# SamsungLabs/nb-asr

Measured on AMD Instinct MI355X. Metric: utterances_per_sec, higher is better.
Workload: dtype f32

## Files before the change

### include/nbasr.h

```cpp
#ifndef NBASR_H
#define NBASR_H

#include <stddef.h>

#ifdef __cplusplus
extern "C" {
#endif

#define NBASR_ABI_VERSION 6

#define NBASR_OK 0
#define NBASR_EINVAL (-1)
#define NBASR_EALIGN (-2)
#define NBASR_ENULL (-3)

typedef void* nbasr_stream_t;

#define NBASR_F32 0
#define NBASR_BF16 1

int nbasr_version(void);

const char* nbasr_build_id(void);

// ... 11 lines not shown
    const float* beta;
} nbasr_deferred_ln;

int nbasr_layernorm_channels(const void* x, const float* gamma, const float* beta, void* y, float* absmax,
                             int batch, int channels, int frames, int ld, float eps, int in_dtype, int out_dtype,
                             nbasr_stream_t stream);

int nbasr_dense_conv1d_fused(const float* x, const float* w, const float* bias,
                             const float* skip0, const float* skip1, const float* skip2,
                             float* y, int batch, int c_in, int frames_in, int ld_in,
                             int c_out, int ld_out, int kernel, int stride,
                             const nbasr_deferred_ln* ln, int ln_on_x, int ln_on_skip0, nbasr_stream_t stream);

#define NBASR_DENSE_STATS_UNIT 16
#define NBASR_DENSE_BF16X3 0
#define NBASR_DENSE_F16X2 1
#define NBASR_DENSE_BF16 2
size_t nbasr_packed_dense_weights_bytes(int scheme, int c_out, int c_in, int kernel, int row_tile);
int nbasr_pack_dense_weights(int scheme, const float* w, void* packed, int c_out, int c_in, int kernel, int stride, int row_tile,
                             nbasr_stream_t stream);
int nbasr_dense_conv1d_packed(int scheme, const void* x, int x_is_image, const float* x_absmax, const float* x_range,
                              const void* packed_w, const float* bias,
                              const float* skip0, const float* skip1, const float* skip2, void* y,
                              int batch, int c_in, int frames_in, int ld_in, int c_out, int ld_out, int kernel, int stride,
                              int row_tile, int frame_tile, const nbasr_deferred_ln* ln, float* stats_part, nbasr_stream_t stream);
int nbasr_input_range(const float* x, float* range, int batch, int channels, int frames, int ld, nbasr_stream_t stream);

size_t nbasr_split_image_bytes(int batch, int channels, int ld);
int nbasr_layernorm_split_image(const float* x, const float* gamma, const float* beta, float* stats, float* bound,
                                void* image, int batch, int channels, int frames, int ld, float eps,
                                nbasr_stream_t stream);
int nbasr_split_image_ranged(const float* x, const float* x_range, void* image, int batch, int channels, int frames, int ld,
                             nbasr_stream_t stream);

int nbasr_lstm_input_projection(const float* x, const float* w_ih, const float* b_ih, const float* b_hh,
                                float* gates_ws, int batch, int c_in, int frames, int ld, int hidden,
                                const nbasr_deferred_ln* ln, nbasr_stream_t stream);
size_t nbasr_lstm_packed_whh_bytes(int hidden);
int nbasr_lstm_pack_whh(const float* w_hh, void* packed, int hidden, nbasr_stream_t stream);
int nbasr_lstm_recurrence_packed(const float* gates_ws, const void* packed_whh, float* cell_ws, float* h_out,
                                 int batch, int frames, int hidden, nbasr_stream_t stream);
#define NBASR_LSTM_SEQ_INJECT_FAULT 1
size_t nbasr_lstm_seq_workspace_bytes(int batch, int hidden);
int nbasr_lstm_recurrence_seq(const float* gates_ws, const void* packed_whh, float* cell_ws, float* h_out, void* seq_ws,
                              int batch, int frames, int hidden, int flags, nbasr_stream_t stream);
int nbasr_lstm_seq_status(const void* seq_ws, nbasr_stream_t stream);
size_t nbasr_lstm_packed_whh16_bytes(int hidden);
int nbasr_lstm_pack_whh16(const float* w_hh, void* packed, int hidden, nbasr_stream_t stream);
size_t nbasr_lstm_xcd_workspace_bytes(int batch, int hidden);
int nbasr_lstm_recurrence_xcd(const float* gates_ws, const void* packed_whh16, float* cell_ws, float* h_out, void* xcd_ws,
                              int batch, int frames, int hidden, int flags, nbasr_stream_t stream);
int nbasr_lstm_recurrence_frames16(const float* gates_ws, const void* packed_whh16, float* cell_ws, float* h_out, void* xcd_ws,
                                   int batch, int frames, int hidden, nbasr_stream_t stream);
#define NBASR_LSTM_CONTINUE 2
int nbasr_lstm_recurrence_frames16_state(const float* gates_ws, const void* packed_whh16, float* cell_ws, float* h_out, void* xcd_ws,
                                         const float* h0, int batch, int frames, int hidden, int flags, nbasr_stream_t stream);

int nbasr_linear_head(const float* h, const float* w, const float* bias, float* logits,
                      int rows, int features, int classes, nbasr_stream_t stream);

int nbasr_linear_head_bct(const float* x, const float* w, const float* bias, float* logits,
                          int batch, int features, int frames, int ld, int classes,
                          const nbasr_deferred_ln* ln, nbasr_stream_t stream);

int nbasr_channel_stats(const void* x, float* stats, int batch, int channels, int frames, int ld, float eps, int dtype,
                        nbasr_stream_t stream);
// ... 141 lines not shown
```

### nb_asr_amd/csrc/layernorm.hip

```cpp
#include "storage.h"

namespace nbasr {

constexpr int LN_ROWS = 16;
constexpr int LN_QS = 16;

template <typename T, bool MINMAX = false, int FR = Chunk<T>::FR>
__device__ __forceinline__ void tile_statistics(const T* x, int channels, int ld, float eps, size_t base, bool active,
                                                int row, int ql, float (*s_mean)[LN_QS * FR], float (*s_m2)[LN_QS * FR],
                                                float* s_cnt, float* s_mu, float* s_rstd,
                                                float (*s_lo)[LN_QS * FR] = nullptr, float (*s_hi)[LN_QS * FR] = nullptr)
{
    float shift[FR], s1[FR], s2[FR], lo[FR], hi[FR];
#pragma unroll
    for (int r = 0; r < FR; ++r) { shift[r] = 0.f; s1[r] = 0.f; s2[r] = 0.f; lo[r] = 3.0e38f; hi[r] = -3.0e38f; }
    int n = 0;
    if (active && row < channels) {
        load_frames<FR>(x + base + static_cast<size_t>(row) * ld, shift);
        auto fold = [&](const float (&e)[FR]) {
#pragma unroll
            for (int r = 0; r < FR; ++r) {
                const float d = e[r] - shift[r];
                s1[r] += d;
                s2[r] = __builtin_fmaf(d, d, s2[r]);
// ... 158 lines not shown
    NBASR_REQUIRE(x && gamma && beta && y, NBASR_ENULL, "%s: NULL pointer", what);
    NBASR_REQUIRE(aligned16(x) && aligned16(y), NBASR_EALIGN, "%s: x, y must be 16-byte aligned", what);
    NBASR_REQUIRE(batch <= 65535, NBASR_EINVAL, "%s: batch %d > 65535", what, batch);
    NBASR_REQUIRE(!absmax || in_dtype == NBASR_F32, NBASR_EINVAL, "%s: the absmax by-product exists for fp32 tensors only", what);
    const int nq = ld / fr;
    const dim3 grid((nq + LN_QS - 1) / LN_QS, batch);
    if (in_dtype == NBASR_BF16) {
        if (out_dtype == NBASR_BF16)
            hipLaunchKernelGGL((layernorm_channels_kernel<bf16_t, bf16_t, false>), grid, dim3(256), 0, as_stream(stream),
                               static_cast<const bf16_t*>(x), gamma, beta, static_cast<bf16_t*>(y), channels, frames, ld, eps, static_cast<unsigned*>(nullptr));
        else
            hipLaunchKernelGGL((layernorm_channels_kernel<bf16_t, float, false>), grid, dim3(256), 0, as_stream(stream),
                               static_cast<const bf16_t*>(x), gamma, beta, static_cast<float*>(y), channels, frames, ld, eps, static_cast<unsigned*>(nullptr));
    } else if (absmax) {
        zero_async(absmax, sizeof(float) * batch, as_stream(stream));
        hipLaunchKernelGGL((layernorm_channels_kernel<float, float, true>), grid, dim3(256), 0, as_stream(stream),
                           static_cast<const float*>(x), gamma, beta, static_cast<float*>(y), channels, frames, ld, eps, reinterpret_cast<unsigned*>(absmax));
    } else {
        hipLaunchKernelGGL((layernorm_channels_kernel<float, float, false>), grid, dim3(256), 0, as_stream(stream),
                           static_cast<const float*>(x), gamma, beta, static_cast<float*>(y), channels, frames, ld, eps, static_cast<unsigned*>(nullptr));
    }
    return launch_status(what);
}

extern "C" int nbasr_layernorm_channels(const void* x, const float* gamma, const float* beta, void* y, float* absmax, int batch,
                                        int channels, int frames, int ld, float eps, int in_dtype, int out_dtype, nbasr_stream_t stream)
{
    clear_error();
    NBASR_REQUIRE(!absmax || (in_dtype == NBASR_F32 && out_dtype == NBASR_F32), NBASR_EINVAL,
                  "nbasr_layernorm_channels: the max|y| by-product exists for fp32 -> fp32 only");
    return layernorm_impl("nbasr_layernorm_channels", x, gamma, beta, y, absmax, batch, channels, frames, ld, eps, stream, in_dtype, out_dtype);
}

__global__ __launch_bounds__(256) void channel_stats_bound_kernel(const float* __restrict__ x, const float* __restrict__ gamma,
                                                                  const float* __restrict__ beta, float* __restrict__ stats,
                                                                  unsigned* __restrict__ bound, int channels, int frames, int ld, float eps)
{
    __shared__ float s_mean[LN_ROWS][LN_QS * 4];
    __shared__ float s_m2[LN_ROWS][LN_QS * 4];
    __shared__ float s_cnt[LN_ROWS];
    __shared__ float s_mu[LN_QS * 4];
    __shared__ float s_rstd[LN_QS * 4];
    __shared__ float s_gb[8];
    __shared__ float s_lo[LN_ROWS][LN_QS * 4];
    __shared__ float s_hi[LN_ROWS][LN_QS * 4];

    const int ql = threadIdx.x & (LN_QS - 1);
    const int row = threadIdx.x / LN_QS;
    const int nq = ld >> 2;
    const int q = blockIdx.x * LN_QS + ql;
    const int b = blockIdx.y;
    const bool active = q < nq;
    const size_t base = static_cast<size_t>(b) * channels * ld + static_cast<size_t>(q) * 4;

    float gm = 0.f, bm = 0.f;
    for (int c = threadIdx.x; c < channels; c += 256) { gm = fmaxf(gm, fabsf(gamma[c])); bm = fmaxf(bm, fabsf(beta[c])); }
#pragma unroll
    for (int d = 32; d >= 1; d >>= 1) { gm = fmaxf(gm, __shfl_xor(gm, d)); bm = fmaxf(bm, __shfl_xor(bm, d)); }
    if ((threadIdx.x & 63) == 0) { s_gb[threadIdx.x >> 6] = gm; s_gb[4 + (threadIdx.x >> 6)] = bm; }

    tile_statistics<float, true>(x, channels, ld, eps, base, active, row, ql, s_mean, s_m2, s_cnt, s_mu, s_rstd, s_lo, s_hi);
    gm = fmaxf(fmaxf(s_gb[0], s_gb[1]), fmaxf(s_gb[2], s_gb[3]));
    bm = fmaxf(fmaxf(s_gb[4], s_gb[5]), fmaxf(s_gb[6], s_gb[7]));

    float dev = 0.f;
    if (threadIdx.x < LN_QS * 4) {
        const int t = blockIdx.x * (LN_QS * 4) + threadIdx.x;
        if (t < ld) {
            const bool live = t < frames;
            float* srow = stats + static_cast<size_t>(b) * 2 * ld;
            srow[t] = live ? s_mu[threadIdx.x] : 0.f;
            srow[ld + t] = live ? s_rstd[threadIdx.x] : 0.f;
            if (live) dev = finite_abs(fmaxf(s_hi[0][threadIdx.x] - s_mu[threadIdx.x], s_mu[threadIdx.x] - s_lo[0][threadIdx.x]) * s_rstd[threadIdx.x]);
        }
    }
    if (threadIdx.x < 64) {
#pragma unroll
        for (int d = 32; d >= 1; d >>= 1) dev = fmaxf(dev, __shfl_xor(dev, d));
        if (threadIdx.x == 0) atomicMax(bound + b, __float_as_uint(finite_abs((dev * gm + bm) * 1.0001f)));
    }
}

template <bool NORM>
__global__ __launch_bounds__(256) void normalize_split_kernel(const float* __restrict__ x, const float* __restrict__ stats,
                                                              const float* __restrict__ gamma, const float* __restrict__ beta,
                                                              const float* __restrict__ bound, unsigned char* __restrict__ image,
                                                              int channels, int , int ld,
                                                              int bound_stride)
{
    typedef _Float16 halfx8 __attribute__((ext_vector_type(8)));
    const int ql = threadIdx.x & 63, oct0 = (threadIdx.x >> 6) + 4 * blockIdx.z;
    const int nq = ld >> 2;
    const int q = blockIdx.x * 64 + ql;
    const int b = blockIdx.y;
    const int n_groups = (channels + 15) >> 4;
    const size_t rows = static_cast<size_t>(ld) + 1;
    unsigned char* const img_b = image + static_cast<size_t>(b) * n_groups * 4 * rows * 16;
    if (blockIdx.x == 0 && blockIdx.z == 0) {
        const uint4 z = make_uint4(0u, 0u, 0u, 0u);
        for (int pl = threadIdx.x; pl < n_groups * 4; pl += 256) *reinterpret_cast<uint4*>(img_b + static_cast<size_t>(pl) * rows * 16) = z;
    }
    if (q >= nq) return;
    float scale = 1.f;
    {
        const unsigned bits = __float_as_uint(bound[static_cast<size_t>(b) * bound_stride]);
        const int e = static_cast<int>((bits >> 23) & 0xffu);
        int k = (bits & 0x7fffffffu) ? (127 + 14) - e : 0;
        k = k > 126 ? 126 : (k < -126 ? -126 : k);
        scale = __uint_as_float(static_cast<unsigned>(127 + k) << 23);
    }
    float m4[4] = {0.f, 0.f, 0.f, 0.f}, r4[4] = {0.f, 0.f, 0.f, 0.f};
    if constexpr (NORM) {
        const float* st = stats + static_cast<size_t>(b) * 2 * ld + q * 4;
        const float4 mu = *reinterpret_cast<const float4*>(st), rs = *reinterpret_cast<const float4*>(st + ld);
        m4[0] = mu.x; m4[1] = mu.y; m4[2] = mu.z; m4[3] = mu.w;
        r4[0] = rs.x; r4[1] = rs.y; r4[2] = rs.z; r4[3] = rs.w;
    }
    const float* xb = x + static_cast<size_t>(b) * channels * ld + static_cast<size_t>(q) * 4;
    const int n_oct = (channels + 7) >> 3;
    for (int oct = oct0; oct < 2 * n_groups; oct += 4 * gridDim.z) {
        float v[8][4];
#pragma unroll
        for (int c = 0; c < 8; ++c) {
            const int ch = oct * 8 + c;
            float4 t4 = make_float4(0.f, 0.f, 0.f, 0.f);
            float g = 0.f, be = 0.f;
            if (oct < n_oct && ch < channels) {
                t4 = *reinterpret_cast<const float4*>(xb + static_cast<size_t>(ch) * ld);
                if constexpr (NORM) { g = gamma[ch]; be = beta[ch]; }
            }
            const float e4[4] = {t4.x, t4.y, t4.z, t4.w};
#pragma unroll
            for (int r = 0; r < 4; ++r) {
                if constexpr (NORM) v[c][r] = (ch < channels) ? ln_apply(e4[r], m4[r], r4[r], g, be) * scale : 0.f;
                else                v[c][r] = e4[r] * scale;
            }
        }
        unsigned char* plane_hi = img_b + ((static_cast<size_t>(oct >> 1) * 4 + (oct & 1)) * rows + 1 + static_cast<size_t>(q) * 4) * 16;
        unsigned char* plane_lo = plane_hi + 2 * rows * 16;
#pragma unroll
        for (int r = 0; r < 4; ++r) {
            halfx8 hi, lo;
#pragma unroll
            for (int c = 0; c < 8; ++c) {
                const _Float16 h = static_cast<_Float16>(v[c][r]);
                hi[c] = h;
                lo[c] = static_cast<_Float16>(v[c][r] - static_cast<float>(h));
            }
            *reinterpret_cast<halfx8*>(plane_hi + r * 16) = hi;
            *reinterpret_cast<halfx8*>(plane_lo + r * 16) = lo;
        }
    }
}

static int split_grid_z(int tiles, int batch)
{
    const long long wgs = static_cast<long long>(tiles) * batch;
    int z = 4;
    while (z < 16 && wgs * z < 512) z *= 2;
    return z;
}

extern "C" int nbasr_layernorm_split_image(const float* x, const float* gamma, const float* beta, float* stats, float* bound,
                                           void* image, int batch, int channels, int frames, int ld, float eps,
                                           nbasr_stream_t stream)
{
    clear_error();
    NBASR_REQUIRE(batch >= 0 && channels > 0 && frames >= 0, NBASR_EINVAL, "nbasr_layernorm_split_image: bad sizes");
    NBASR_REQUIRE(ld >= frames && ld % 4 == 0, NBASR_EALIGN, "nbasr_layernorm_split_image: ld=%d must be >= frames=%d and a multiple of 4", ld, frames);
    if (batch == 0 || ld == 0) return NBASR_OK;
    NBASR_REQUIRE(x && gamma && beta && stats && bound && image, NBASR_ENULL, "nbasr_layernorm_split_image: NULL pointer");
    NBASR_REQUIRE(aligned16(x) && aligned16(stats) && aligned16(image), NBASR_EALIGN, "nbasr_layernorm_split_image: x, stats, image must be 16-byte aligned");
    NBASR_REQUIRE(batch <= 65535, NBASR_EINVAL, "nbasr_layernorm_split_image: batch %d > 65535", batch);
    zero_async(bound, sizeof(float) * batch, as_stream(stream));
    const int nq = ld / 4;
    hipLaunchKernelGGL(channel_stats_bound_kernel, dim3((nq + LN_QS - 1) / LN_QS, batch), dim3(256), 0, as_stream(stream),
                       x, gamma, beta, stats, reinterpret_cast<unsigned*>(bound), channels, frames, ld, eps);
    hipLaunchKernelGGL(normalize_split_kernel<true>, dim3((nq + 63) / 64, batch, split_grid_z((nq + 63) / 64, batch)), dim3(256), 0, as_stream(stream),
                       x, stats, gamma, beta, bound, static_cast<unsigned char*>(image), channels, frames, ld, 1);
    return launch_status("nbasr_layernorm_split_image");
}

__global__ __launch_bounds__(256) void input_range_kernel(const float* __restrict__ x, unsigned* __restrict__ range,
                                                          int channels, int frames, int ld)
{
    __shared__ float s_max[4][256];
    __shared__ unsigned s_bad[4];
    const int b = blockIdx.y;
    const int lane = threadIdx.x & 63, slice = threadIdx.x >> 6;
    const int t0 = (blockIdx.x * 64 + lane) * 4;
    float m[4] = {0.f, 0.f, 0.f, 0.f};
    unsigned bad = 0u;
    if (t0 < frames) {
        const float* col = x + static_cast<size_t>(b) * channels * ld + t0;
        const bool whole = t0 + 4 <= ld && ld % 4 == 0 && (reinterpret_cast<size_t>(x) & 15) == 0;
        for (int c = slice; c < channels; c += 4) {
            float v[4] = {0.f, 0.f, 0.f, 0.f};
            if (whole) {
                const float4 q = *reinterpret_cast<const float4*>(col + static_cast<size_t>(c) * ld);
                v[0] = q.x; v[1] = q.y; v[2] = q.z; v[3] = q.w;
            } else {
#pragma unroll
                for (int r = 0; r < 4; ++r) if (t0 + r < frames) v[r] = col[static_cast<size_t>(c) * ld + r];
            }
#pragma unroll
            for (int r = 0; r < 4; ++r) {
                const float a = fabsf(v[r]);
                if (t0 + r < frames) {
                    if (!(a <= 3.4028234664e38f)) bad = 1u;
                    else m[r] = fmaxf(m[r], a);
                }
            }
        }
// ... 24 lines not shown
    const int b = blockIdx.x * blockDim.x + threadIdx.x;
    if (b < batch) { range[4 * b] = 0u; range[4 * b + 1] = 0x7f800000u; range[4 * b + 2] = 0u; range[4 * b + 3] = 0u; }
}

extern "C" int nbasr_input_range(const float* x, float* range, int batch, int channels, int frames, int ld, nbasr_stream_t stream)
{
    clear_error();
    NBASR_REQUIRE(batch >= 0 && channels > 0 && frames >= 0 && ld >= frames, NBASR_EINVAL, "nbasr_input_range: bad sizes");
    if (batch == 0) return NBASR_OK;
    NBASR_REQUIRE(range, NBASR_ENULL, "nbasr_input_range: range is NULL");
    NBASR_REQUIRE(batch <= 65535, NBASR_EINVAL, "nbasr_input_range: batch %d > 65535", batch);
    hipLaunchKernelGGL(input_range_init_kernel, dim3((batch + 255) / 256), dim3(256), 0, as_stream(stream), reinterpret_cast<unsigned*>(range), batch);
    if (frames > 0) {
        NBASR_REQUIRE(x, NBASR_ENULL, "nbasr_input_range: x is NULL");
        hipLaunchKernelGGL(input_range_kernel, dim3((frames + 255) / 256, batch), dim3(256), 0, as_stream(stream), x,
                           reinterpret_cast<unsigned*>(range), channels, frames, ld);
    }
    return launch_status("nbasr_input_range");
}

extern "C" int nbasr_split_image_ranged(const float* x, const float* x_range, void* image, int batch, int channels, int frames,
                                        int ld, nbasr_stream_t stream)
{
    clear_error();
    NBASR_REQUIRE(batch >= 0 && channels > 0 && frames >= 0, NBASR_EINVAL, "nbasr_split_image_ranged: bad sizes");
    NBASR_REQUIRE(ld >= frames && ld % 4 == 0, NBASR_EALIGN, "nbasr_split_image_ranged: ld=%d must be >= frames=%d and a multiple of 4", ld, frames);
    if (batch == 0 || ld == 0) return NBASR_OK;
    NBASR_REQUIRE(x && x_range && image, NBASR_ENULL, "nbasr_split_image_ranged: NULL pointer");
    NBASR_REQUIRE(aligned16(x) && aligned16(image), NBASR_EALIGN, "nbasr_split_image_ranged: x, image must be 16-byte aligned");
    NBASR_REQUIRE(batch <= 65535, NBASR_EINVAL, "nbasr_split_image_ranged: batch %d > 65535", batch);
    const int nq = ld / 4;
    hipLaunchKernelGGL(normalize_split_kernel<false>, dim3((nq + 63) / 64, batch, split_grid_z((nq + 63) / 64, batch)), dim3(256), 0, as_stream(stream),
                       x, static_cast<const float*>(nullptr), static_cast<const float*>(nullptr), static_cast<const float*>(nullptr),
                       x_range, static_cast<unsigned char*>(image), channels, frames, ld, 4);
    return launch_status("nbasr_split_image_ranged");
}

extern "C" int nbasr_channel_stats(const void* x, float* stats, int batch, int channels, int frames, int ld, float eps, int dtype,
                                     nbasr_stream_t stream)
{
    clear_error();
    NBASR_REQUIRE(dtype == NBASR_F32 || dtype == NBASR_BF16, NBASR_EINVAL, "nbasr_channel_stats: unknown dtype %d", dtype);
    NBASR_REQUIRE(batch >= 0 && channels > 0 && frames >= 0, NBASR_EINVAL, "nbasr_channel_stats: bad sizes");
    const int fr = dtype == NBASR_BF16 ? 8 : 4;
    NBASR_REQUIRE(ld >= frames && ld % fr == 0, NBASR_EALIGN, "nbasr_channel_stats: ld=%d must be >= frames=%d and a multiple of %d", ld, frames, fr);
    if (batch == 0 || ld == 0) return NBASR_OK;
    NBASR_REQUIRE(x && stats, NBASR_ENULL, "nbasr_channel_stats: NULL pointer");
    NBASR_REQUIRE(aligned16(x) && aligned16(stats), NBASR_EALIGN, "nbasr_channel_stats: x, stats must be 16-byte aligned");
    NBASR_REQUIRE(batch <= 65535, NBASR_EINVAL, "nbasr_channel_stats: batch %d > 65535", batch);
    const int nq = ld / fr;
    const dim3 grid((nq + LN_QS - 1) / LN_QS, batch);
    if (dtype == NBASR_BF16)
        hipLaunchKernelGGL(channel_stats_kernel<bf16_t>, grid, dim3(256), 0, as_stream(stream), static_cast<const bf16_t*>(x), stats, channels, frames, ld, eps);
    else
        hipLaunchKernelGGL(channel_stats_kernel<float>, grid, dim3(256), 0, as_stream(stream), static_cast<const float*>(x), stats, channels, frames, ld, eps);
    return launch_status("nbasr_channel_stats");
}

template <typename T, bool NORM>
__global__ __launch_bounds__(256) void bf16_image_kernel(const T* __restrict__ x, const float* __restrict__ stats,
                                                         const float* __restrict__ gamma, const float* __restrict__ beta,
                                                         unsigned char* __restrict__ image, int channels, int frames, int ld)
{
    constexpr int FR = Chunk<T>::FR;
    const int ql = threadIdx.x & 15, oct0 = threadIdx.x >> 4;
    const int nq = ld / FR;
    const int q = blockIdx.x * 16 + ql;
// ... 110 lines not shown
```

### nb_asr_amd/executor.py

```python
import collections
import math
import os
import threading
import weakref

import torch

from . import hip


def node_into(node, inputs, frames, out, ln0=None, stats=None, linear_ctx=None, gc_variant=0):
    from .ops import PadConvRelu, Linear, Zero, Identity
    if len(inputs) != len(node.branch_ops):
        raise AssertionError('Branch op and input list have different lenghts')
    skips = [src for branch, src in zip(node.branch_ops, inputs) if isinstance(branch, Identity)]
    op, last = node.op, inputs[-1]
    on_x = ln0 is not None and len(inputs) == 1
    on_s0 = ln0 is not None and isinstance(node.branch_ops[0], Identity)
    ln = ln0 if (on_x or on_s0) else None
    if isinstance(op, PadConvRelu):
        hip.grouped_conv1d_node(last, op.conv.weight.detach(), op.conv.bias.detach(), skips, out, frames,
                                op.groups, op.kernel_size, op.dilation, ln, on_x, on_s0,
                                stats[1] if stats is not None else None, gc_variant)
    elif isinstance(op, Linear):
# ... 347 lines not shown
            self.cell_ws = self._buf('cell', batch * LSTM_HIDDEN)
            self.h_out = self._buf('h_out', batch * self.out_frames * LSTM_HIDDEN)[: batch * self.out_frames * LSTM_HIDDEN] \
                .view(batch, self.out_frames, LSTM_HIDDEN)
        else:
            self.h_out = None

    def _timed(self, kind, meta, launch):
        if self.timer is None:
            return launch()
        start, stop = torch.cuda.Event(enable_timing=True), torch.cuda.Event(enable_timing=True)
        start.record()
        out = launch()
        stop.record()
        self.timer.append((kind, meta, start, stop))
        return out

    def _cached(self, param, tag, build):
        key = (id(param), tag)
        hit = self._packed.get(key)
        if hit is None or hit[0]() is not param or hit[1] != param._version:
            if len(self._packed) >= 512:
                self._packed = {k: v for k, v in self._packed.items() if v[0]() is not None}
            if hit is not None:
                self.wait_tails()
            built = build()
            if self.side_stream is not None and isinstance(built, torch.Tensor):
                built.record_stream(self.side_stream)
            hit = (weakref.ref(param), param._version, built)
            self._packed[key] = hit
            self._tapes.clear()
            self._mutations += 1
        return hit[2]

    def _packed_weights(self, layer, scheme, row_tile=128):
        w = layer.conv.weight
        return self._cached(w, (scheme, row_tile, layer.strides), lambda: hip.pack_dense_weights(w.detach(), layer.strides, scheme, row_tile))

    def _row_tile(self, c_out, frames_out, allow_64=True):
        n_nt = (hip.round_up4(frames_out) + 255) // 256

        def cost(rows):
            wgs = -(-c_out // rows) * n_nt * self.batch
            return -(-wgs // 256) * rows
        rows = 160 if cost(160) < cost(128) else 128
        score = float(cost(rows))
        if allow_64:
            for r, margin in ((96, 1.1), (64, 1.25)):
                if margin * cost(r) < score:
                    rows, score = r, margin * cost(r)
        return rows

    def _bf16_tile(self, c_out, frames_out, pipe=False):
        forced = os.environ.get('NBASR_BF16_FTILE')
        best = None
        for rows in (128, 160):
            for ftile in ((int(forced),) if forced else (256,) if pipe else (256, 512)):
                wgs = -(-c_out // rows) * -(-hip.row_pitch(frames_out, torch.bfloat16) // ftile) * self.batch
                cost = -(-wgs // 256) * rows * ftile * (0.9 if ftile == 512 else 1.0)
                if best is None or cost < best[0]:
                    best = (cost, rows, ftile)
        return best[1], best[2]

    def _dense_tile(self, layer, frames_out):
        conv = layer.conv
        rows = self._row_tile(conv.out_channels, frames_out)
        best = (rows, 256)
# ... 53 lines not shown
                                                         layer.kernel_size, layer.conv.bias.detach(), out, layer.strides, rows, part, ftile)
        if self.dense_mode != 'f32' and layer.kernel_size == 8:
            scheme = 'f16x2' if self.dense_mode == 'auto' and absmax is not None and ln is None else 'bf16x3'
            self.dense_schemes[blk] = scheme
            part = None
            if want_stats:
                part = self._conv_part = self._dense_part(layer.conv.out_channels, out.shape[2])
            return hip.dense_conv1d_fused_packed(act, act_frames, self._packed_weights(layer, scheme), layer.conv.out_channels,
                                                 layer.kernel_size, layer.conv.bias.detach(), (), out, layer.strides, ln, scheme,
                                                 absmax if scheme == 'f16x2' else None, part)
        self.dense_schemes[blk] = 'f32'
        return hip.dense_conv1d_fused(act, act_frames, layer.conv.weight.detach(), layer.conv.bias.detach(), (), out,
                                      layer.strides, ln, ln is not None, False)

    @staticmethod
    def _cheap_consumer(nxt):
        from .model import SearchCell
        from .ops import Linear
        return isinstance(nxt, SearchCell) and not isinstance(nxt.nodes[0].op, Linear)

    def _norm(self, norm, act, act_frames, kind_meta, taps, tap_idx, nxt, out=None, defer=None):
        if defer is None:
            defer = self._cheap_consumer(nxt)
        if not defer or out is not None:
            dst = act if out is None else out
            from .ops import PadConvRelu
            want_range = self.dense_mode == 'auto' and isinstance(nxt, PadConvRelu) and nxt.groups == 1 and nxt.kernel_size == 8
            if want_range and taps is None and out is None:
                b, c, ld = act.shape
                image = self._buf('image', max(hip.load_library().nbasr_split_image_bytes(b, c, ld), 16), torch.uint8)
                self._stat_turn ^= 1
                stats = self.stats[self._stat_turn][: b * 2 * ld].view(b, 2, ld)
                bound = self.absmax[:b]
                self._timed('layernorm', kind_meta, lambda: hip.layernorm_split_image(act, norm.weight.detach(), norm.bias.detach(),
                                                                                   stats, bound, image, act_frames, norm.eps))
                self._act_image = (image, bound)
                self._act_absmax = None
                return None
            absmax = self.absmax[: act.shape[0]] if want_range else None
            self._timed('layernorm', kind_meta, lambda: hip.layernorm_channels(act, norm.weight.detach(), norm.bias.detach(),
                                                                               dst, act_frames, norm.eps, absmax))
            self._act_absmax = absmax
            return None
        self._stat_turn ^= 1
        b, _, ld = act.shape
        stats = self.stats[self._stat_turn][: b * 2 * ld].view(b, 2, ld)
        conv_part, self._conv_part = self._conv_part, None
        if conv_part is not None:
            c = act.shape[1]
            self._timed('stats_finalize', kind_meta, lambda: hip.grouped_stats_finalize(conv_part, stats, c, act_frames, c, norm.eps, hip.DENSE_STATS_UNIT))
        else:
            self._timed('channel_stats', kind_meta, lambda: hip.channel_stats(act, stats, act_frames, norm.eps))
        if taps is not None:
            copy = torch.empty_like(act)
            hip.layernorm_channels(act, norm.weight.detach(), norm.bias.detach(), copy, act_frames, norm.eps)
            taps[tap_idx] = copy[:, :, :act_frames].clone()
        return (stats, norm.weight.detach(), norm.bias.detach())

    def _gc_variant(self, view, node=None, ln0=None, stats=None, n_inputs=0):
        forced = os.environ.get('NBASR_GC_F32_VARIANT')
        if forced is not None:
            v = int(forced)
            return (v & ~hip.GC_OSPLIT if v & hip.GC_PIPE else 0) if (v & hip.GC_OSPLIT and (stats is not None or node is None)) else v
        if node is None or not self.gc_table:
            return 0
        op = node.op
        groups = getattr(op, 'groups', 0)
        if not groups:
# ... 745 lines not shown
```

### nb_asr_amd/hip.py

```python
import ctypes
import os
import threading
import pathlib

import torch

LIB_PATH = pathlib.Path(__file__).resolve().parent / 'lib' / 'libnbasr_hip.so'
ABI_VERSION = 6

_c_float_p = ctypes.c_void_p
_c_int = ctypes.c_int
_c_stream = ctypes.c_void_p

class DeferredLN(ctypes.Structure):
    _fields_ = [('stats', ctypes.c_void_p), ('gamma', ctypes.c_void_p), ('beta', ctypes.c_void_p)]


_c_ln_p = ctypes.POINTER(DeferredLN)

SIGNATURES = {
    'nbasr_version': (_c_int, []),
    'nbasr_build_id': (ctypes.c_char_p, []),
    'nbasr_last_error': (ctypes.c_char_p, []),
    'nbasr_pad_amounts': (_c_int, [_c_int, _c_int, _c_int, ctypes.POINTER(_c_int), ctypes.POINTER(_c_int)]),
    'nbasr_output_frames': (_c_int, [_c_int]),
    'nbasr_stream_create': (_c_int, [ctypes.POINTER(ctypes.c_void_p)]),
    'nbasr_layernorm_channels': (_c_int, [_c_float_p] * 5 + [_c_int] * 4 + [ctypes.c_float, _c_int, _c_int, _c_stream]),
    'nbasr_channel_stats': (_c_int, [_c_float_p] * 2 + [_c_int] * 4 + [ctypes.c_float, _c_int, _c_stream]),
    'nbasr_grouped_stats_workspace_bytes': (ctypes.c_size_t, [_c_int] * 3),
    'nbasr_grouped_stats_finalize': (_c_int, [_c_float_p] * 2 + [_c_int] * 6 + [ctypes.c_float, _c_stream]),
    'nbasr_grouped_conv1d_node': (_c_int, [_c_float_p] * 7 + [_c_int] * 7 + [_c_ln_p, _c_int, _c_int, _c_float_p, _c_int, _c_int, _c_stream]),
    'nbasr_pack_grouped_weights': (_c_int, [_c_float_p] * 2 + [_c_int] * 3 + [_c_stream]),
    'nbasr_grouped_cell_fits': (_c_int, [_c_int] * 3),
    'nbasr_grouped_cell_fused': (_c_int, [_c_float_p, _c_float_p, _c_float_p, _c_int, _c_int, _c_float_p, _c_float_p, _c_int, _c_int,
                                          _c_float_p, _c_float_p, _c_int, _c_int, _c_int, _c_float_p] + [_c_int] * 5 + [_c_ln_p, _c_float_p, _c_int, _c_stream]),
    'nbasr_grouped_cell_mfma_weights_bytes': (ctypes.c_size_t, [_c_int] * 3),
    'nbasr_grouped_cell_mfma_pack': (_c_int, [_c_float_p] * 2 + [_c_int] * 3 + [_c_stream]),
    'nbasr_grouped_cell_mfma_fits': (_c_int, [_c_int] * 3),
    'nbasr_grouped_cell_mfma': (_c_int, [_c_float_p, _c_float_p, _c_float_p, _c_int, _c_int, _c_float_p, _c_float_p, _c_int, _c_int,
                                         _c_float_p, _c_float_p, _c_int, _c_int, _c_int, _c_float_p] + [_c_int] * 5 + [_c_ln_p, _c_stream]),
    'nbasr_skip_sum': (_c_int, [_c_float_p] * 4 + [_c_int] * 4 + [_c_ln_p, _c_int, _c_int, _c_stream]),
    'nbasr_repitch': (_c_int, [_c_float_p] * 2 + [_c_int] * 5 + [_c_stream]),
    'nbasr_convert': (_c_int, [_c_float_p] * 2 + [ctypes.c_longlong, _c_int, _c_int, _c_stream]),
    'nbasr_dense_conv1d_fused': (_c_int, [_c_float_p] * 7 + [_c_int] * 8 + [_c_ln_p, _c_int, _c_int, _c_stream]),
    'nbasr_packed_dense_weights_bytes': (ctypes.c_size_t, [_c_int] * 5),
    'nbasr_pack_dense_weights': (_c_int, [_c_int] + [_c_float_p] * 2 + [_c_int] * 5 + [_c_stream]),
    'nbasr_dense_conv1d_packed': (_c_int, [_c_int, _c_float_p, _c_int] + [_c_float_p] * 8 + [_c_int] * 10 + [_c_ln_p, _c_float_p, _c_stream]),
    'nbasr_input_range': (_c_int, [_c_float_p] * 2 + [_c_int] * 4 + [_c_stream]),
    'nbasr_split_image_bytes': (ctypes.c_size_t, [_c_int] * 3),
    'nbasr_layernorm_split_image': (_c_int, [_c_float_p] * 6 + [_c_int] * 4 + [ctypes.c_float, _c_stream]),
    'nbasr_split_image_ranged': (_c_int, [_c_float_p] * 3 + [_c_int] * 4 + [_c_stream]),
    'nbasr_bf16_image_bytes': (ctypes.c_size_t, [_c_int] * 3),
    'nbasr_bf16_image': (_c_int, [_c_float_p] * 5 + [_c_int] * 4 + [ctypes.c_float, _c_int, _c_stream]),
    'nbasr_pointwise_packed_weights_bytes': (ctypes.c_size_t, [_c_int] * 2),
    'nbasr_pointwise_workspace_bytes': (ctypes.c_size_t, [_c_int] * 3),
    'nbasr_pack_pointwise_weights': (_c_int, [_c_float_p] * 2 + [_c_int] * 2 + [_c_stream]),
    'nbasr_linear_fused_packed': (_c_int, [_c_float_p] * 8 + [_c_int] * 5 + [_c_ln_p, _c_int, _c_int, _c_stream]),
    'nbasr_pointwise_linear': (_c_int, [_c_float_p] * 4 + [_c_int] * 6 + [_c_stream]),
    'nbasr_lstm_input_projection': (_c_int, [_c_float_p] * 5 + [_c_int] * 5 + [_c_ln_p, _c_stream]),
    'nbasr_lstm_input_projection_packed': (_c_int, [_c_float_p] * 6 + [_c_int] * 5 + [_c_ln_p, _c_stream]),
    'nbasr_lstm_input_projection_packed_into': (_c_int, [_c_float_p] * 6 + [_c_int] * 5 + [_c_ln_p, _c_int, _c_int, _c_stream]),
    'nbasr_pointwise_bf16_weights_bytes': (ctypes.c_size_t, [_c_int] * 2),
    'nbasr_pointwise_bf16_workspace_bytes': (ctypes.c_size_t, [_c_int] * 3),
    'nbasr_pack_pointwise_weights_bf16': (_c_int, [_c_float_p] * 2 + [_c_int] * 2 + [_c_stream]),
    'nbasr_linear_fused_bf16': (_c_int, [_c_float_p] * 8 + [_c_int] * 5 + [_c_ln_p, _c_int, _c_int, _c_stream]),
    'nbasr_lstm_input_projection_bf16': (_c_int, [_c_float_p] * 6 + [_c_int] * 5 + [_c_ln_p, _c_stream]),
    'nbasr_lstm_packed_whh_bytes': (ctypes.c_size_t, [_c_int]),
    'nbasr_lstm_pack_whh': (_c_int, [_c_float_p] * 2 + [_c_int, _c_stream]),
    'nbasr_lstm_recurrence_packed': (_c_int, [_c_float_p] * 4 + [_c_int] * 3 + [_c_stream]),
    'nbasr_lstm_seq_workspace_bytes': (ctypes.c_size_t, [_c_int] * 2),
    'nbasr_lstm_recurrence_seq': (_c_int, [_c_float_p] * 5 + [_c_int] * 4 + [_c_stream]),
    'nbasr_lstm_seq_status': (_c_int, [_c_float_p, _c_stream]),
    'nbasr_lstm_packed_whh16_bytes': (ctypes.c_size_t, [_c_int]),
    'nbasr_lstm_pack_whh16': (_c_int, [_c_float_p] * 2 + [_c_int, _c_stream]),
    'nbasr_lstm_xcd_workspace_bytes': (ctypes.c_size_t, [_c_int] * 2),
    'nbasr_lstm_recurrence_xcd': (_c_int, [_c_float_p] * 5 + [_c_int] * 4 + [_c_stream]),
    'nbasr_lstm_recurrence_frames16': (_c_int, [_c_float_p] * 5 + [_c_int] * 3 + [_c_stream]),
    'nbasr_lstm_recurrence_frames16_state': (_c_int, [_c_float_p] * 6 + [_c_int] * 4 + [_c_stream]),
    'nbasr_linear_head': (_c_int, [_c_float_p] * 4 + [_c_int] * 3 + [_c_stream]),
    'nbasr_linear_head_bct': (_c_int, [_c_float_p] * 4 + [_c_int] * 5 + [_c_ln_p, _c_stream]),
    'nbasr_ctc_postprocess': (_c_int, [_c_float_p] * 5 + [_c_int] * 4 + [_c_stream]),
    'nbasr_ctc_greedy_stream': (_c_int, [_c_float_p] * 4 + [_c_int] * 4 + [_c_stream]),
    'nbasr_ctc_loss': (_c_int, [_c_float_p] * 5 + [_c_int] * 6 + [_c_stream]),
    'nbasr_ctc_grad_workspace_bytes': (ctypes.c_size_t, [_c_int] * 3),
# ... 250 lines not shown
                                         _act(y, 'y'), b, c, frames, ld, _ln(ln), int(ln_on_skip0), dtype_code(dt), _stream(y)),
           'nbasr_skip_sum')
    return y


def channel_stats(x, stats, frames, eps):
    b, c, ld = x.shape
    _check(load_library().nbasr_channel_stats(_act(x, 'x'), _dev(stats, 'stats'), b, c, frames, ld, float(eps), dtype_code(x.dtype),
                                              _stream(x)), 'nbasr_channel_stats')
    return stats


def layernorm_channels(x, gamma, beta, y, frames, eps, absmax=None):
    b, c, ld = x.shape
    if absmax is not None and absmax.numel() != b:
        raise HipError('absmax must hold one float per utterance')
    _check(load_library().nbasr_layernorm_channels(_act(x, 'x'), _dev(gamma, 'gamma'), _dev(beta, 'beta'), _act(y, 'y'),
                                                   _opt(absmax, 'absmax'), b, c, frames, ld, float(eps), dtype_code(x.dtype),
                                                   dtype_code(y.dtype), _stream(x)), 'nbasr_layernorm_channels')
    return y


def split_image(batch, channels, ld, device):
    return torch.empty(max(load_library().nbasr_split_image_bytes(batch, channels, ld), 16), dtype=torch.uint8, device=device)


def layernorm_split_image(x, gamma, beta, stats, bound, image, frames, eps):
    b, c, ld = x.shape
    if image.dtype != torch.uint8 or image.numel() < load_library().nbasr_split_image_bytes(b, c, ld):
        raise HipError('image buffer too small: allocate it with split_image(batch, channels, ld, device)')
    _check(load_library().nbasr_layernorm_split_image(_dev(x, 'x'), _dev(gamma, 'gamma'), _dev(beta, 'beta'), _dev(stats, 'stats'),
                                                      _dev(bound, 'bound'), image.data_ptr(), b, c, frames, ld, float(eps), _stream(x)),
           'nbasr_layernorm_split_image')
    return image


def dense_conv1d_fused_packed_f16_img(image, bound, batch, c_in, frames_in, ld_in, packed, c_out, kernel, bias, y, stride,
                                      row_tile=128, stats_part=None, frame_tile=256):
    _check_packed(packed, 'f16x2', c_out, c_in, kernel, row_tile)
    if image.numel() < load_library().nbasr_split_image_bytes(batch, c_in, ld_in):
        raise HipError('image buffer too small for (batch, c_in, ld_in)')
    return _dense_packed('f16x2', image.data_ptr(), True, bound, None, packed, bias, (None, None, None), y, _dev(y, 'y'), batch, c_in,
                         frames_in, ld_in, c_out, kernel, stride, row_tile, None, _stream(y), stats_part, frame_tile)


def input_range(x, frames, out):
    b, c, ld = x.shape
    if out.numel() < 4 * b:
        raise HipError('input_range: out needs 4 floats per utterance')
    _check(load_library().nbasr_input_range(_dev(x, 'x'), _dev(out, 'range'), b, c, frames, ld, _stream(x)), 'nbasr_input_range')
    return out


def dense_conv1d_first_ranged(x, frames_in, x_range, packed_f16, packed_bf16x3, c_out, kernel, bias, y, stride, image=None, row_tile=128,
                              stats_part=None, frame_tile=256):
    lib = load_library()
    b, c_in, ld_in = x.shape
    _check_packed(packed_f16, 'f16x2', c_out, c_in, kernel, 128 if image is None else row_tile)
    _check_packed(packed_bf16x3, 'bf16x3', c_out, c_in, kernel)
    none3, stream = (None, None, None), _stream(x)
    if image is not None:
        if image.dtype != torch.uint8 or image.numel() < lib.nbasr_split_image_bytes(b, c_in, ld_in):
            raise HipError('dense_conv1d_first_ranged: image workspace too small (nbasr_split_image_bytes)')
        _check(lib.nbasr_split_image_ranged(_dev(x, 'x'), _dev(x_range, 'x_range'), image.data_ptr(), b, c_in, frames_in, ld_in, stream),
               'nbasr_split_image_ranged')
    if image is not None:
# ... 800 lines not shown
```

Baseline: 11230.

## Tile layernorm split-image: cached param max, per-tile bounds, XCD-contiguous grid, prefetch

Adds a tiled variant of the layernorm-to-split-image path. The per-block gamma/beta absmax scan is replaced by a cached two-float result that is recomputed only when the parameters change. Per-tile bounds go to a workspace instead of a zero fill plus atomicMax, and the normalize kernel reduces them itself. Both kernels move to 1-D grids remapped so that consecutive work lands on the same XCD, and the normalize loop software-prefetches the next octet of rows. The cost is extra register pressure, a serial bound reduction in every normalize block, and cache-invalidation logic on the host.

```diff
diff --git a/include/nbasr.h b/include/nbasr.h
--- a/include/nbasr.h
+++ b/include/nbasr.h
@@ -67,6 +67,11 @@
                                 nbasr_stream_t stream);
 int nbasr_split_image_ranged(const float* x, const float* x_range, void* image, int batch, int channels, int frames, int ld,
                              nbasr_stream_t stream);
+int nbasr_layernorm_param_max(const float* gamma, const float* beta, float* gb_max, int channels, nbasr_stream_t stream);
+size_t nbasr_layernorm_split_ws_bytes(int batch, int ld);
+int nbasr_layernorm_split_image_tiled(const float* x, const float* gamma, const float* beta, const float* gb_max, float* stats,
+                                      float* bound, float* tile_ws, void* image, int batch, int channels, int frames, int ld,
+                                      float eps, nbasr_stream_t stream);
 
 int nbasr_lstm_input_projection(const float* x, const float* w_ih, const float* b_ih, const float* b_hh,
                                 float* gates_ws, int batch, int c_in, int frames, int ld, int hidden,
diff --git a/nb_asr_amd/csrc/layernorm.hip b/nb_asr_amd/csrc/layernorm.hip
--- a/nb_asr_amd/csrc/layernorm.hip
+++ b/nb_asr_amd/csrc/layernorm.hip
@@ -214,9 +214,18 @@
     return layernorm_impl("nbasr_layernorm_channels", x, gamma, beta, y, absmax, batch, channels, frames, ld, eps, stream, in_dtype, out_dtype);
 }
 
+
+__device__ __forceinline__ unsigned xcd_contiguous(unsigned id, unsigned n)
+{
+    const unsigned per = n >> 3, rem = n & 7u, k = id & 7u;
+    return k * per + (k < rem ? k : rem) + (id >> 3);
+}
+
+template <bool TILED>
 __global__ __launch_bounds__(256) void channel_stats_bound_kernel(const float* __restrict__ x, const float* __restrict__ gamma,
                                                                   const float* __restrict__ beta, float* __restrict__ stats,
-                                                                  unsigned* __restrict__ bound, int channels, int frames, int ld, float eps)
+                                                                  unsigned* __restrict__ bound, int channels, int frames, int ld, float eps,
+                                                                  const float* __restrict__ gb_max, float* __restrict__ tile_bound, int n_tiles)
 {
     __shared__ float s_mean[LN_ROWS][LN_QS * 4];
     __shared__ float s_m2[LN_ROWS][LN_QS * 4];
@@ -230,24 +239,35 @@
     const int ql = threadIdx.x & (LN_QS - 1);
     const int row = threadIdx.x / LN_QS;
     const int nq = ld >> 2;
-    const int q = blockIdx.x * LN_QS + ql;
-    const int b = blockIdx.y;
+    int tile = blockIdx.x, b = blockIdx.y;
+    if constexpr (TILED) {
+        const unsigned w = xcd_contiguous(blockIdx.x, gridDim.x);
+        tile = static_cast<int>(w % static_cast<unsigned>(n_tiles));
+        b = static_cast<int>(w / static_cast<unsigned>(n_tiles));
+    }
+    const int q = tile * LN_QS + ql;
     const bool active = q < nq;
     const size_t base = static_cast<size_t>(b) * channels * ld + static_cast<size_t>(q) * 4;
 
     float gm = 0.f, bm = 0.f;
-    for (int c = threadIdx.x; c < channels; c += 256) { gm = fmaxf(gm, fabsf(gamma[c])); bm = fmaxf(bm, fabsf(beta[c])); }
-#pragma unroll
-    for (int d = 32; d >= 1; d >>= 1) { gm = fmaxf(gm, __shfl_xor(gm, d)); bm = fmaxf(bm, __shfl_xor(bm, d)); }
-    if ((threadIdx.x & 63) == 0) { s_gb[threadIdx.x >> 6] = gm; s_gb[4 + (threadIdx.x >> 6)] = bm; }
+    if constexpr (!TILED) {
+        for (int c = threadIdx.x; c < channels; c += 256) { gm = fmaxf(gm, fabsf(gamma[c])); bm = fmaxf(bm, fabsf(beta[c])); }
+#pragma unroll
+        for (int d = 32; d >= 1; d >>= 1) { gm = fmaxf(gm, __shfl_xor(gm, d)); bm = fmaxf(bm, __shfl_xor(bm, d)); }
+        if ((threadIdx.x & 63) == 0) { s_gb[threadIdx.x >> 6] = gm; s_gb[4 + (threadIdx.x >> 6)] = bm; }
+    }
 
     tile_statistics<float, true>(x, channels, ld, eps, base, active, row, ql, s_mean, s_m2, s_cnt, s_mu, s_rstd, s_lo, s_hi);
-    gm = fmaxf(fmaxf(s_gb[0], s_gb[1]), fmaxf(s_gb[2], s_gb[3]));
-    bm = fmaxf(fmaxf(s_gb[4], s_gb[5]), fmaxf(s_gb[6], s_gb[7]));
+    if constexpr (TILED) {
+        gm = gb_max[0]; bm = gb_max[1];
+    } else {
+        gm = fmaxf(fmaxf(s_gb[0], s_gb[1]), fmaxf(s_gb[2], s_gb[3]));
+        bm = fmaxf(fmaxf(s_gb[4], s_gb[5]), fmaxf(s_gb[6], s_gb[7]));
+    }
 
     float dev = 0.f;
     if (threadIdx.x < LN_QS * 4) {
-        const int t = blockIdx.x * (LN_QS * 4) + threadIdx.x;
+        const int t = tile * (LN_QS * 4) + threadIdx.x;
         if (t < ld) {
             const bool live = t < frames;
             float* srow = stats + static_cast<size_t>(b) * 2 * ld;
@@ -259,33 +279,52 @@
     if (threadIdx.x < 64) {
 #pragma unroll
         for (int d = 32; d >= 1; d >>= 1) dev = fmaxf(dev, __shfl_xor(dev, d));
-        if (threadIdx.x == 0) atomicMax(bound + b, __float_as_uint(finite_abs((dev * gm + bm) * 1.0001f)));
-    }
-}
-
-template <bool NORM>
+        if (threadIdx.x == 0) {
+            const float tb = finite_abs((dev * gm + bm) * 1.0001f);
+            if constexpr (TILED) tile_bound[static_cast<size_t>(b) * n_tiles + tile] = tb;
+            else                 atomicMax(bound + b, __float_as_uint(tb));
+        }
+    }
+}
+
+template <bool NORM, bool TILED = false>
 __global__ __launch_bounds__(256) void normalize_split_kernel(const float* __restrict__ x, const float* __restrict__ stats,
                                                               const float* __restrict__ gamma, const float* __restrict__ beta,
                                                               const float* __restrict__ bound, unsigned char* __restrict__ image,
                                                               int channels, int , int ld,
-                                                              int bound_stride)
+                                                              int bound_stride, float* __restrict__ bound_out, int n_bound, int tiles_x, int tiles_z)
 {
     typedef _Float16 halfx8 __attribute__((ext_vector_type(8)));
-    const int ql = threadIdx.x & 63, oct0 = (threadIdx.x >> 6) + 4 * blockIdx.z;
+    int bx = blockIdx.x, b = blockIdx.y, bz = blockIdx.z, nz = gridDim.z;
+    if constexpr (TILED) {
+        unsigned w = xcd_contiguous(blockIdx.x, gridDim.x);
+        nz = tiles_z;
+        bz = static_cast<int>(w % static_cast<unsigned>(tiles_z)); w /= static_cast<unsigned>(tiles_z);
+        bx = static_cast<int>(w % static_cast<unsigned>(tiles_x));
+        b = static_cast<int>(w / static_cast<unsigned>(tiles_x));
+    }
+    const int ql = threadIdx.x & 63, oct0 = (threadIdx.x >> 6) + 4 * bz;
     const int nq = ld >> 2;
-    const int q = blockIdx.x * 64 + ql;
-    const int b = blockIdx.y;
+    const int q = bx * 64 + ql;
     const int n_groups = (channels + 15) >> 4;
     const size_t rows = static_cast<size_t>(ld) + 1;
     unsigned char* const img_b = image + static_cast<size_t>(b) * n_groups * 4 * rows * 16;
-    if (blockIdx.x == 0 && blockIdx.z == 0) {
+    float bnd;
+    if constexpr (TILED) {
+        bnd = 0.f;
+        for (int i = 0; i < n_bound; ++i) bnd = fmaxf(bnd, bound[static_cast<size_t>(b) * n_bound + i]);
+    } else {
+        bnd = bound[static_cast<size_t>(b) * bound_stride];
+    }
+    if (bx == 0 && bz == 0) {
         const uint4 z = make_uint4(0u, 0u, 0u, 0u);
         for (int pl = threadIdx.x; pl < n_groups * 4; pl += 256) *reinterpret_cast<uint4*>(img_b + static_cast<size_t>(pl) * rows * 16) = z;
+        if constexpr (TILED) { if (threadIdx.x == 0) bound_out[b] = bnd; }
     }
     if (q >= nq) return;
     float scale = 1.f;
     {
-        const unsigned bits = __float_as_uint(bound[static_cast<size_t>(b) * bound_stride]);
+        const unsigned bits = __float_as_uint(bnd);
         const int e = static_cast<int>((bits >> 23) & 0xffu);
         int k = (bits & 0x7fffffffu) ? (127 + 14) - e : 0;
         k = k > 126 ? 126 : (k < -126 ? -126 : k);
@@ -300,18 +339,22 @@
     }
     const float* xb = x + static_cast<size_t>(b) * channels * ld + static_cast<size_t>(q) * 4;
     const int n_oct = (channels + 7) >> 3;
-    for (int oct = oct0; oct < 2 * n_groups; oct += 4 * gridDim.z) {
-        float v[8][4];
+    auto fetch = [&](int oct, float4 (&t4)[8]) {
 #pragma unroll
         for (int c = 0; c < 8; ++c) {
             const int ch = oct * 8 + c;
-            float4 t4 = make_float4(0.f, 0.f, 0.f, 0.f);
+            t4[c] = make_float4(0.f, 0.f, 0.f, 0.f);
+            if (oct < n_oct && ch < channels) t4[c] = *reinterpret_cast<const float4*>(xb + static_cast<size_t>(ch) * ld);
+        }
+    };
+    auto emit = [&](int oct, const float4 (&t4)[8]) {
+        float v[8][4];
+#pragma unroll
+        for (int c = 0; c < 8; ++c) {
+            const int ch = oct * 8 + c;
             float g = 0.f, be = 0.f;
-            if (oct < n_oct && ch < channels) {
-                t4 = *reinterpret_cast<const float4*>(xb + static_cast<size_t>(ch) * ld);
-                if constexpr (NORM) { g = gamma[ch]; be = beta[ch]; }
-            }
-            const float e4[4] = {t4.x, t4.y, t4.z, t4.w};
+            if constexpr (NORM) { if (oct < n_oct && ch < channels) { g = gamma[ch]; be = beta[ch]; } }
+            const float e4[4] = {t4[c].x, t4[c].y, t4[c].z, t4[c].w};
 #pragma unroll
             for (int r = 0; r < 4; ++r) {
                 if constexpr (NORM) v[c][r] = (ch < channels) ? ln_apply(e4[r], m4[r], r4[r], g, be) * scale : 0.f;
@@ -331,6 +374,26 @@
             }
             *reinterpret_cast<halfx8*>(plane_hi + r * 16) = hi;
             *reinterpret_cast<halfx8*>(plane_lo + r * 16) = lo;
+        }
+    };
+    const int step = 4 * nz, end = 2 * n_groups;
+    if constexpr (TILED) {
+        float4 cur[8], nxt[8];
+        if (oct0 < end) fetch(oct0, cur);
+        for (int oct = oct0; oct < end; oct += step) {
+            const bool more = oct + step < end;
+            if (more) fetch(oct + step, nxt);
+            emit(oct, cur);
+            if (more) {
+#pragma unroll
+                for (int c = 0; c < 8; ++c) cur[c] = nxt[c];
+            }
+        }
+    } else {
+        for (int oct = oct0; oct < end; oct += step) {
+            float4 t4[8];
+            fetch(oct, t4);
+            emit(oct, t4);
         }
     }
 }
@@ -356,11 +419,68 @@
     NBASR_REQUIRE(batch <= 65535, NBASR_EINVAL, "nbasr_layernorm_split_image: batch %d > 65535", batch);
     zero_async(bound, sizeof(float) * batch, as_stream(stream));
     const int nq = ld / 4;
-    hipLaunchKernelGGL(channel_stats_bound_kernel, dim3((nq + LN_QS - 1) / LN_QS, batch), dim3(256), 0, as_stream(stream),
-                       x, gamma, beta, stats, reinterpret_cast<unsigned*>(bound), channels, frames, ld, eps);
+    hipLaunchKernelGGL(channel_stats_bound_kernel<false>, dim3((nq + LN_QS - 1) / LN_QS, batch), dim3(256), 0, as_stream(stream),
+                       x, gamma, beta, stats, reinterpret_cast<unsigned*>(bound), channels, frames, ld, eps,
+                       static_cast<const float*>(nullptr), static_cast<float*>(nullptr), 0);
     hipLaunchKernelGGL(normalize_split_kernel<true>, dim3((nq + 63) / 64, batch, split_grid_z((nq + 63) / 64, batch)), dim3(256), 0, as_stream(stream),
-                       x, stats, gamma, beta, bound, static_cast<unsigned char*>(image), channels, frames, ld, 1);
+                       x, stats, gamma, beta, bound, static_cast<unsigned char*>(image), channels, frames, ld, 1,
+                       static_cast<float*>(nullptr), 0, 0, 0);
     return launch_status("nbasr_layernorm_split_image");
+}
+
+__global__ __launch_bounds__(256) void layernorm_param_max_kernel(const float* __restrict__ gamma, const float* __restrict__ beta,
+                                                                  float* __restrict__ gb_max, int channels)
+{
+    __shared__ float s_gb[8];
+    float gm = 0.f, bm = 0.f;
+    for (int c = threadIdx.x; c < channels; c += 256) { gm = fmaxf(gm, fabsf(gamma[c])); bm = fmaxf(bm, fabsf(beta[c])); }
+#pragma unroll
+    for (int d = 32; d >= 1; d >>= 1) { gm = fmaxf(gm, __shfl_xor(gm, d)); bm = fmaxf(bm, __shfl_xor(bm, d)); }
+    if ((threadIdx.x & 63) == 0) { s_gb[threadIdx.x >> 6] = gm; s_gb[4 + (threadIdx.x >> 6)] = bm; }
+    __syncthreads();
+    if (threadIdx.x == 0) {
+        gb_max[0] = fmaxf(fmaxf(s_gb[0], s_gb[1]), fmaxf(s_gb[2], s_gb[3]));
+        gb_max[1] = fmaxf(fmaxf(s_gb[4], s_gb[5]), fmaxf(s_gb[6], s_gb[7]));
+    }
+}
+
+extern "C" int nbasr_layernorm_param_max(const float* gamma, const float* beta, float* gb_max, int channels, nbasr_stream_t stream)
+{
+    clear_error();
+    NBASR_REQUIRE(channels > 0, NBASR_EINVAL, "nbasr_layernorm_param_max: bad sizes");
+    NBASR_REQUIRE(gamma && beta && gb_max, NBASR_ENULL, "nbasr_layernorm_param_max: NULL pointer");
+    hipLaunchKernelGGL(layernorm_param_max_kernel, dim3(1), dim3(256), 0, as_stream(stream), gamma, beta, gb_max, channels);
+    return launch_status("nbasr_layernorm_param_max");
+}
+
+extern "C" size_t nbasr_layernorm_split_ws_bytes(int batch, int ld)
+{
+    if (batch <= 0 || ld <= 0) return 0;
+    return static_cast<size_t>(batch) * ((ld / 4 + LN_QS - 1) / LN_QS) * sizeof(float);
+}
+
+extern "C" int nbasr_layernorm_split_image_tiled(const float* x, const float* gamma, const float* beta, const float* gb_max, float* stats,
+                                                 float* bound, float* tile_ws, void* image, int batch, int channels, int frames, int ld,
+                                                 float eps, nbasr_stream_t stream)
+{
+    clear_error();
+    NBASR_REQUIRE(batch >= 0 && channels > 0 && frames >= 0, NBASR_EINVAL, "nbasr_layernorm_split_image_tiled: bad sizes");
+    NBASR_REQUIRE(ld >= frames && ld % 4 == 0, NBASR_EALIGN, "nbasr_layernorm_split_image_tiled: ld=%d must be >= frames=%d and a multiple of 4", ld, frames);
+    if (batch == 0 || ld == 0) return NBASR_OK;
+    NBASR_REQUIRE(x && gamma && beta && gb_max && stats && bound && tile_ws && image, NBASR_ENULL, "nbasr_layernorm_split_image_tiled: NULL pointer");
+    NBASR_REQUIRE(aligned16(x) && aligned16(stats) && aligned16(image), NBASR_EALIGN, "nbasr_layernorm_split_image_tiled: x, stats, image must be 16-byte aligned");
+    NBASR_REQUIRE(batch <= 65535, NBASR_EINVAL, "nbasr_layernorm_split_image_tiled: batch %d > 65535", batch);
+    const int nq = ld / 4;
+    const int n_tiles = (nq + LN_QS - 1) / LN_QS, tiles_x = (nq + 63) / 64, tiles_z = split_grid_z(tiles_x, batch);
+    NBASR_REQUIRE(static_cast<long long>(n_tiles) * batch <= 0x7fffffffLL && static_cast<long long>(tiles_x) * tiles_z * batch <= 0x7fffffffLL,
+                  NBASR_EINVAL, "nbasr_layernorm_split_image_tiled: too many tiles");
+    hipLaunchKernelGGL(channel_stats_bound_kernel<true>, dim3(static_cast<unsigned>(n_tiles) * batch), dim3(256), 0, as_stream(stream),
+                       x, gamma, beta, stats, static_cast<unsigned*>(nullptr), channels, frames, ld, eps, gb_max, tile_ws, n_tiles);
+    const dim3 grid(static_cast<unsigned>(tiles_x) * tiles_z * batch);
+    unsigned char* img = static_cast<unsigned char*>(image);
+    hipLaunchKernelGGL((normalize_split_kernel<true, true>), grid, dim3(256), 0, as_stream(stream),
+                       x, stats, gamma, beta, tile_ws, img, channels, frames, ld, 1, bound, n_tiles, tiles_x, tiles_z);
+    return launch_status("nbasr_layernorm_split_image_tiled");
 }
 
 __global__ __launch_bounds__(256) void input_range_kernel(const float* __restrict__ x, unsigned* __restrict__ range,
@@ -451,7 +571,7 @@
     const int nq = ld / 4;
     hipLaunchKernelGGL(normalize_split_kernel<false>, dim3((nq + 63) / 64, batch, split_grid_z((nq + 63) / 64, batch)), dim3(256), 0, as_stream(stream),
                        x, static_cast<const float*>(nullptr), static_cast<const float*>(nullptr), static_cast<const float*>(nullptr),
-                       x_range, static_cast<unsigned char*>(image), channels, frames, ld, 4);
+                       x_range, static_cast<unsigned char*>(image), channels, frames, ld, 4, static_cast<float*>(nullptr), 0, 0, 0);
     return launch_status("nbasr_split_image_ranged");
 }
 
diff --git a/nb_asr_amd/executor.py b/nb_asr_amd/executor.py
--- a/nb_asr_amd/executor.py
+++ b/nb_asr_amd/executor.py
@@ -403,6 +403,19 @@
             self._mutations += 1
         return hit[2]
 
+    def _ln_param_max(self, norm):
+        w, bias = norm.weight, norm.bias
+
+        def build():
+            return (weakref.ref(bias), bias._version, hip.layernorm_param_max(w.detach(), bias.detach()))
+        hit = self._cached(w, 'ln_param_max', build)
+        if hit[0]() is not bias or hit[1] != bias._version:
+            del self._packed[(id(w), 'ln_param_max')]
+            hit = self._cached(w, 'ln_param_max', build)
+        if self.side_stream is not None:
+            hit[2].record_stream(self.side_stream)
+        return hit[2]
+
     def _packed_weights(self, layer, scheme, row_tile=128):
         w = layer.conv.weight
         return self._cached(w, (scheme, row_tile, layer.strides), lambda: hip.pack_dense_weights(w.detach(), layer.strides, scheme, row_tile))
@@ -522,8 +535,10 @@
                 self._stat_turn ^= 1
                 stats = self.stats[self._stat_turn][: b * 2 * ld].view(b, 2, ld)
                 bound = self.absmax[:b]
-                self._timed('layernorm', kind_meta, lambda: hip.layernorm_split_image(act, norm.weight.detach(), norm.bias.detach(),
-                                                                                   stats, bound, image, act_frames, norm.eps))
+                gb_max = self._ln_param_max(norm)
+                tile_ws = self._buf('ln_tile_bound', max(hip.load_library().nbasr_layernorm_split_ws_bytes(b, ld) // 4, 4))
+                self._timed('layernorm', kind_meta, lambda: hip.layernorm_split_image_tiled(act, norm.weight.detach(), norm.bias.detach(), gb_max,
+                                                                                         stats, bound, tile_ws, image, act_frames, norm.eps))
                 self._act_image = (image, bound)
                 self._act_absmax = None
                 return None
diff --git a/nb_asr_amd/hip.py b/nb_asr_amd/hip.py
--- a/nb_asr_amd/hip.py
+++ b/nb_asr_amd/hip.py
@@ -50,6 +50,9 @@
     'nbasr_split_image_bytes': (ctypes.c_size_t, [_c_int] * 3),
     'nbasr_layernorm_split_image': (_c_int, [_c_float_p] * 6 + [_c_int] * 4 + [ctypes.c_float, _c_stream]),
     'nbasr_split_image_ranged': (_c_int, [_c_float_p] * 3 + [_c_int] * 4 + [_c_stream]),
+    'nbasr_layernorm_param_max': (_c_int, [_c_float_p] * 3 + [_c_int, _c_stream]),
+    'nbasr_layernorm_split_ws_bytes': (ctypes.c_size_t, [_c_int] * 2),
+    'nbasr_layernorm_split_image_tiled': (_c_int, [_c_float_p] * 8 + [_c_int] * 4 + [ctypes.c_float, _c_stream]),
     'nbasr_bf16_image_bytes': (ctypes.c_size_t, [_c_int] * 3),
     'nbasr_bf16_image': (_c_int, [_c_float_p] * 5 + [_c_int] * 4 + [ctypes.c_float, _c_int, _c_stream]),
     'nbasr_pointwise_packed_weights_bytes': (ctypes.c_size_t, [_c_int] * 2),
@@ -366,6 +369,26 @@
     _check(load_library().nbasr_layernorm_split_image(_dev(x, 'x'), _dev(gamma, 'gamma'), _dev(beta, 'beta'), _dev(stats, 'stats'),
                                                       _dev(bound, 'bound'), image.data_ptr(), b, c, frames, ld, float(eps), _stream(x)),
            'nbasr_layernorm_split_image')
+    return image
+
+
+def layernorm_param_max(gamma, beta):
+    out = torch.empty(2, dtype=torch.float32, device=gamma.device)
+    _check(load_library().nbasr_layernorm_param_max(_dev(gamma, 'gamma'), _dev(beta, 'beta'), _dev(out, 'gb_max'), gamma.numel(),
+                                                    _stream(gamma)), 'nbasr_layernorm_param_max')
+    return out
+
+
+def layernorm_split_image_tiled(x, gamma, beta, gb_max, stats, bound, tile_ws, image, frames, eps):
+    b, c, ld = x.shape
+    lib = load_library()
+    if image.dtype != torch.uint8 or image.numel() < lib.nbasr_split_image_bytes(b, c, ld):
+        raise HipError('image buffer too small: allocate it with split_image(batch, channels, ld, device)')
+    if tile_ws.numel() * 4 < lib.nbasr_layernorm_split_ws_bytes(b, ld) or gb_max.numel() < 2:
+        raise HipError('layernorm_split_image_tiled: tile_ws / gb_max too small')
+    _check(lib.nbasr_layernorm_split_image_tiled(_dev(x, 'x'), _dev(gamma, 'gamma'), _dev(beta, 'beta'), _dev(gb_max, 'gb_max'),
+                                                 _dev(stats, 'stats'), _dev(bound, 'bound'), _dev(tile_ws, 'tile_ws'), image.data_ptr(),
+                                                 b, c, frames, ld, float(eps), _stream(x)), 'nbasr_layernorm_split_image_tiled')
     return image
 
 
```

Result: no change. 11250 (median of 4 runs) (+0.2%).
